# rgcgithub/regenie

Measured on AMD Instinct MI355X. Metric: Step-1 SNPs x samples x phenos / sec, higher is better.
Workload: dtype fp4 (exact integer Gram) + i8 (exact fixed-point digit planes of the fp64 operands: G~X / G~Y, many-row predictions) + f64 (solves, level 1); 1 GPU; BASELINE configs[1]: synthetic PLINK bed 50000 samples x 100000 SNPs (100000 per GPU), 1 QT pheno, bsize 1000, 22 chromosomes, 5-fold CV, 5x5 ridge grid; `value` is the HBM-resident figure (packed genotypes generated on the device, timed region = level 0 + level 1 + LOCO rows); the complete run from files on disk is `end_to_end_from_files`; samples=50000, snps=100000, phenos=1, bsize=1000, blocks=109, parallelism=blocks sharded x1, all-gather of W, level-1 Gram tiles / ridge systems shared x1

## Files before the change

### regenie_amd/csrc/l1.hip

```cpp
#include <algorithm>
#include <climits>
#include <cmath>
#include <cstdint>
#include <vector>
#include "rg_internal.h"

#define CT 64

struct L1Rows {
  const double* W; const double* y; const double* zero;
  int64_t Np; int L, P, p, n64;
};
__device__ __forceinline__ const double* l1_row(const L1Rows& R, int row) {
  if (row < R.L) return R.W + ((int64_t)row * R.P + R.p) * R.Np;
  if (row == R.n64) return R.y;
  return R.zero;
}

struct L1G64 {
  L1Rows R; int T, rtot, nslice, ntile, world, rank;
  double* out; int64_t slice_stride;
};
__global__ __launch_bounds__(256, 2) void k_l1_gram64(L1G64 g, SegLayout seg) {
  const int lane = threadIdx.x & 63, wave = threadIdx.x >> 6;
  const int f = blockIdx.y;
  const int item = blockIdx.x * 4 + wave;
  if (item >= g.ntile * g.nslice) return;
  const int sl = item / g.ntile, idx = item % g.ntile;
  if (idx % g.world != g.rank) return;
  int tc = 0, rem = idx;
  while (rem >= g.T + 1 - tc) { rem -= g.T + 1 - tc; ++tc; }
  const int tr = tc + rem;
  const int i = lane & 15, q = lane >> 4;
  const int64_t nch = seg.plen[f] / 64;
  const int64_t c0 = nch * sl / g.nslice, c1 = nch * (sl + 1) / g.nslice;
  const int64_t p0 = seg.pos_start[f] + 2 * q;
  const double* A[4];
  const double* B[4];
#pragma unroll
  for (int m = 0; m < 4; ++m) {
    A[m] = l1_row(g.R, tr * CT + m * 16 + i) + p0;
    B[m] = l1_row(g.R, tc * CT + m * 16 + i) + p0;
  }
  v4d acc[4][4];
// ... 93 lines not shown
    if (s + 1 < ns) issue((s + 1) & 1);
    if (live) {
      double2 a[4][2], b[4][2];
#pragma unroll
      for (int m = 0; m < 4; ++m) {
        a[m][0] = *reinterpret_cast<const double2*>(cur + oa + m * 2048);
        a[m][1] = *reinterpret_cast<const double2*>(cur + oa + m * 2048 + o4);
        b[m][0] = *reinterpret_cast<const double2*>(cur + ob + m * 2048);
        b[m][1] = *reinterpret_cast<const double2*>(cur + ob + m * 2048 + o4);
      }
#pragma unroll
      for (int kk = 0; kk < 4; ++kk)
#pragma unroll
        for (int m = 0; m < 4; ++m)
#pragma unroll
          for (int n = 0; n < 4; ++n) {
            const double av = kk == 0 ? a[m][0].x : (kk == 1 ? a[m][0].y : (kk == 2 ? a[m][1].x : a[m][1].y));
            const double bv = kk == 0 ? b[n][0].x : (kk == 1 ? b[n][0].y : (kk == 2 ? b[n][1].x : b[n][1].y));
            acc[m][n] = __builtin_amdgcn_mfma_f64_16x16x4f64(av, bv, acc[m][n], 0, 0, 0);
          }
    }
    asm volatile("s_waitcnt vmcnt(0) lgkmcnt(0)\n\ts_barrier" ::: "memory");
  }
  if (!live) return;
  double* O = g.out + (int64_t)it.slice * g.slice_stride + (int64_t)f * g.rtot * n64 + (int64_t)row0 * n64 + col0;
#pragma unroll
  for (int m = 0; m < 4; ++m)
#pragma unroll
    for (int n = 0; n < 4; ++n)
#pragma unroll
      for (int r = 0; r < 4; ++r) O[(int64_t)(m * 16 + q + 4 * r) * n64 + n * 16 + i] = acc[m][n][r];
}

__global__ __launch_bounds__(256) void k_l1_wty(L1Rows R, SegLayout seg, int rtot, int world, int rank, double* out) {
  __shared__ double red[4];
  const int l = blockIdx.x, f = blockIdx.y;
  if (l % world != rank) return;
  const double* w = R.W + ((int64_t)l * R.P + R.p) * R.Np + seg.pos_start[f];
  const double* y = R.y + seg.pos_start[f];
  const int64_t n = seg.plen[f];
  double t0 = 0.0, t1 = 0.0;
  for (int64_t e = 2 * (int64_t)threadIdx.x; e < n; e += 512) {
    const double2 wv = *reinterpret_cast<const double2*>(w + e), yv = *reinterpret_cast<const double2*>(y + e);
    t0 = fma(wv.x, yv.x, t0);
    t1 = fma(wv.y, yv.y, t1);
  }
  double t = t0 + t1;
  for (int o = 32; o > 0; o >>= 1) t += __shfl_down(t, o);
  if ((threadIdx.x & 63) == 0) red[threadIdx.x >> 6] = t;
  __syncthreads();
  if (threadIdx.x == 0) out[(int64_t)f * rtot * R.n64 + (int64_t)R.n64 * R.n64 + l] = (red[0] + red[1]) + (red[2] + red[3]);
}

static std::vector<L1Item> l1_build_items(int n64, int K, int nslice, int world, int rank) {
  const int T2 = (n64 + 127) / 128, S = 4, TS = (T2 + S - 1) / S;
  std::vector<std::vector<L1Item>> xl(8);
  int gi = 0;
  for (int f = 0; f < K; ++f)
    for (int sl = 0; sl < nslice; ++sl)
      for (int Mr = 0; Mr < TS; ++Mr)
        for (int Mc = 0; Mc <= Mr; ++Mc) {
          std::vector<L1Item>& dst = xl[gi % 8];
          bool any = false;
          for (int mr = Mr * S; mr < std::min(T2, (Mr + 1) * S); ++mr)
            for (int mc = Mc * S; mc < std::min(T2, (Mc + 1) * S); ++mc) {
              if (mc > mr) continue;
              if ((mr * (mr + 1) / 2 + mc) % world != rank) continue;
              dst.push_back(L1Item{(int16_t)mr, (int16_t)mc, (int16_t)f, (int16_t)sl});
              any = true;
            }
          if (any) ++gi;
        }
  size_t mx = 0;
  for (auto& v : xl) mx = std::max(mx, v.size());
  std::vector<L1Item> items(mx * 8, L1Item{0, 0, -1, 0});
  for (int x = 0; x < 8; ++x)
    for (size_t j = 0; j < xl[x].size(); ++j) items[8 * j + x] = xl[x][j];
  return items;
}

void rg_launch_fold_gram_rows(hipStream_t st, const double* G, int64_t ld, int L, int n64, int rtot, const double* zero,
                              const SegLayout& seg, double* out) {
  L1G64 g;
  g.R = L1Rows{G, zero, zero, ld, L, 1, 0, n64};
  g.T = n64 / CT; g.rtot = rtot; g.nslice = 1; g.ntile = g.T * (g.T + 1) / 2 + g.T; g.world = 1; g.rank = 0;
  g.out = out; g.slice_stride = 0;
  hipLaunchKernelGGL(k_l1_gram64, dim3((g.ntile + 3) / 4, seg.nseg), dim3(256), 0, st, g, seg);
}

__global__ void k_reduce_slices(const double* part, int64_t slice_stride, int nslice, int64_t n, double* out) {
  const int64_t e = (int64_t)blockIdx.x * blockDim.x + threadIdx.x;
  if (e >= n) return;
  double t = 0.0;
  for (int s = 0; s < nslice; ++s) t += part[(int64_t)s * slice_stride + e];
  out[e] = t;
}

__global__ void k_sum_folds(const double* fold, int64_t msz, int nfold, double* sum) {
  const int64_t e = (int64_t)blockIdx.x * blockDim.x + threadIdx.x;
  if (e >= msz) return;
  double t = 0.0;
  for (int f = 0; f < nfold; ++f) t += fold[(int64_t)f * msz + e];
  sum[e] = t;
}

__global__ __launch_bounds__(256) void k_loco(const double* pred, int nchr, int64_t N, const int32_t* chrom, int nchrom,
                                              double* out) {
  const int64_t n = (int64_t)blockIdx.x * 256 + threadIdx.x;
  if (n >= N) return;
  double tot = 0.0;
  for (int k = 0; k < nchr; ++k) tot += pred[(int64_t)k * N + n];
  for (int c = 0; c < nchrom; ++c) out[(int64_t)c * N + n] = tot;
  for (int k = 0; k < nchr; ++k) out[(int64_t)(chrom[k] - 1) * N + n] = tot - pred[(int64_t)k * N + n];
}

int rg_emit_pred(rg_ctx* ctx, hipStream_t st, const double* d_pred, int nchr, int p, double* pred_out) {
  const int64_t N = ctx->N;
  if (ctx->loco_nchrom <= 0) {
    RG_HIP(hipMemcpyAsync(pred_out + (int64_t)p * nchr * N, d_pred, sizeof(double) * (size_t)nchr * N, hipMemcpyDeviceToHost, st));
    return RG_OK;
  }
  if ((int)ctx->loco_chrom.size() != nchr) { ctx->err = "LOCO output: rg_set_loco_output was given a different number of chromosomes"; return RG_ERR_ARG; }
  const int nchrom = ctx->loco_nchrom;
  double* d_out = (double*)rg_ws(ctx, 11, sizeof(double) * (size_t)nchrom * N + sizeof(int32_t) * (size_t)nchr + 64);
  if (!d_out) { ctx->err = "LOCO output: out of device memory"; return RG_ERR_HIP; }
  int32_t* d_chr = reinterpret_cast<int32_t*>(d_out + (size_t)nchrom * N);
  RG_HIP(hipMemcpyAsync(d_chr, ctx->loco_chrom.data(), sizeof(int32_t) * nchr, hipMemcpyHostToDevice, st));
  hipLaunchKernelGGL(k_loco, dim3((unsigned)((N + 255) / 256)), dim3(256), 0, st, d_pred, nchr, N, d_chr, nchrom, d_out);
  RG_HIP(hipMemcpyAsync(pred_out + (int64_t)p * nchrom * N, d_out, sizeof(double) * (size_t)nchrom * N, hipMemcpyDeviceToHost, st));
  return RG_OK;
}

__global__ __launch_bounds__(256) void k_tiles_pack(double* fold, int64_t msz, int T, int n64, double* packed, int unpack) {
  const int t = blockIdx.x, f = blockIdx.y;
  int tr = (int)((sqrtf(8.0f * t + 1.0f) - 1.0f) * 0.5f);
  while ((tr + 1) * (tr + 2) / 2 <= t) ++tr;
  while (tr * (tr + 1) / 2 > t) --tr;
  int tc = t - tr * (tr + 1) / 2;
  if (tr >= T) { tc = t - T * (T + 1) / 2; tr = T; }
  double* src = fold + (int64_t)f * msz + (int64_t)tr * CT * n64 + tc * CT;
  double* pk = packed + ((int64_t)f * gridDim.x + t) * (CT * CT);
  for (int e = threadIdx.x; e < CT * CT; e += 256) {
    const int r = e >> 6, c = e & 63;
    if (unpack) src[(int64_t)r * n64 + c] = pk[e];
    else pk[e] = src[(int64_t)r * n64 + c];
  }
}

#define R1MAX 8
#define L1_CT 256
__global__ __launch_bounds__(256) void k_l1_cv(L1Rows R, const double* alpha , int R1,
                                               const int32_t* chunk_seg, const int64_t* chunk_pos,
                                               const int64_t* chunk_len, double* part) {
  __shared__ double sA[L1_CT][R1MAX];
  __shared__ double sred[4][R1MAX * 3 + 2];
  const int ch = blockIdx.x;
  const int f = chunk_seg[ch];
  const int64_t p0 = chunk_pos[ch], plen = chunk_len[ch];
  double tot[R1MAX * 3 + 2];
#pragma unroll
  for (int t = 0; t < R1MAX * 3 + 2; ++t) tot[t] = 0.0;
  for (int64_t sub = 0; sub < plen; sub += 256) {
// ... 14 lines not shown
        const int cn = min(L1_CT, R.L - c0);
        const double* w = R.W + ((int64_t)c0 * R.P + R.p) * R.Np + pos;
        for (int c = 0; c < cn; ++c) {
          const double x = w[(int64_t)c * R.P * R.Np];
#pragma unroll
          for (int j = 0; j < R1MAX; ++j) acc[j] = fma(x, sA[c][j], acc[j]);
        }
      }
    }
    if (live) {
      const double y = R.y[pos];
#pragma unroll
      for (int j = 0; j < R1MAX; ++j) {
        tot[3 * j] += acc[j];
        tot[3 * j + 1] = fma(acc[j], acc[j], tot[3 * j + 1]);
        tot[3 * j + 2] = fma(acc[j], y, tot[3 * j + 2]);
      }
      tot[R1MAX * 3] += y;
      tot[R1MAX * 3 + 1] = fma(y, y, tot[R1MAX * 3 + 1]);
    }
  }
#pragma unroll
  for (int t = 0; t < R1MAX * 3 + 2; ++t) {
    double x = tot[t];
    for (int o = 32; o > 0; o >>= 1) x += __shfl_down(x, o);
    if ((threadIdx.x & 63) == 0) sred[threadIdx.x >> 6][t] = x;
  }
  __syncthreads();
  if (threadIdx.x < R1MAX * 3 + 2)
    part[(int64_t)ch * (R1MAX * 3 + 2) + threadIdx.x] =
        (sred[0][threadIdx.x] + sred[1][threadIdx.x]) + (sred[2][threadIdx.x] + sred[3][threadIdx.x]);
}

__global__ __launch_bounds__(256) void k_l1_pred(L1Rows R, const double* alpha , int R1,
                                                 int best, const int32_t* chunk_seg,
                                                 const int64_t* chunk_pos, const int64_t* chunk_len,
                                                 const int32_t* chr_col0 , int nchr,
                                                 const int32_t* cidx, int64_t N, double* pred) {
  extern __shared__ double sAl[];
  const int ch = blockIdx.x;
  const int f = chunk_seg[ch];
  const int64_t p0 = chunk_pos[ch], plen = chunk_len[ch];
  const double* al = alpha + ((int64_t)f * R1 + best) * R.n64;
  for (int c = threadIdx.x; c < R.L; c += 256) sAl[c] = al[c];
  __syncthreads();
  for (int64_t sub = 0; sub < plen; sub += 256) {
    const int64_t pos = p0 + sub + threadIdx.x;
    if (sub + threadIdx.x >= plen) continue;
    const int32_t n = cidx[pos];
    if (n < 0) continue;
    for (int c = 0; c < nchr; ++c) {
      double acc = 0.0;
      const double* w = R.W + ((int64_t)chr_col0[c] * R.P + R.p) * R.Np + pos;
      const int nn = chr_col0[c + 1] - chr_col0[c];
      for (int t = 0; t < nn; ++t) acc = fma(w[(int64_t)t * R.P * R.Np], sAl[chr_col0[c] + t], acc);
      pred[(int64_t)c * N + n] = acc;
    }
  }
}

int rg_l1_qt_impl(rg_ctx* ctx, int R1, const double* tau, int nchr, const int32_t* cols_per_chr,
                  double* cumsum_out, int32_t* best_out, double* pred_out) {
  if (!ctx->have_problem || !(ctx->d_W || ctx->v_W)) { ctx->err = "rg_l1_qt: no level-0 predictors"; return RG_ERR_STATE; }
  if (R1 < 1 || R1 > R1MAX) { ctx->err = "rg_l1_qt: n_ridge_l1 must be in [1,8]"; return RG_ERR_ARG; }
  if (ctx->loocv) { ctx->err = "rg_l1_qt: the problem was set up for LOOCV (use rg_l1_qt_loocv)"; return RG_ERR_STATE; }
  hipStream_t st = ctx->stream;
  const int L = ctx->B_total * ctx->R0, K = ctx->K;
  if (!ctx->v_W && ctx->w_nb != ctx->B_total) { ctx->err = "rg_l1_qt: W holds a block range only (rg_set_block_range): level 1 needs the exchanged view"; return RG_ERR_STATE; }
  const double* Wv = ctx->v_W ? ctx->v_W : ctx->d_W;
  const int Pv = ctx->v_W ? ctx->v_np : ctx->P, P = ctx->v_np, p0v = ctx->v_p0;
  int ltot = 0;
  std::vector<int32_t> col0(nchr + 1, 0);
  for (int c = 0; c < nchr; ++c) { col0[c + 1] = col0[c] + cols_per_chr[c]; }
  ltot = col0[nchr];
  if (ltot != L) { ctx->err = "rg_l1_qt: cols_per_chr does not sum to n_blocks*R0"; return RG_ERR_ARG; }
  const int n64 = (int)rg_round_up(L, CT), rtot = n64 + CT, T = n64 / CT;
  const int64_t msz = (int64_t)rtot * n64;
  const int nsys = K * R1;
  const int nch = ctx->n_c256;
  const int NPART = R1MAX * 3 + 2;
  const int world = ctx->coll_world, rank = ctx->coll_rank;
  const bool multi = ctx->coll_allreduce != nullptr;
  const int b0 = multi ? (int)((int64_t)nsys * rank / world) : 0;
  const int b1 = multi ? (int)((int64_t)nsys * (rank + 1) / world) : nsys;
  const int nloc = b1 - b0;
  const int ntile = T * (T + 1) / 2 + T;
  int64_t min_nch = INT64_MAX;
  for (int f = 0; f < K; ++f) min_nch = std::min(min_nch, ctx->seg.plen[f] / 64);
  const int T2 = (n64 + 127) / 128, ntile2 = T2 * (T2 + 1) / 2;
  int nslice = (int)std::min<int64_t>(16, std::max<int64_t>(1, (3072 + (int64_t)ntile2 * K - 1) / ((int64_t)ntile2 * K)));
  nslice = (int)std::max<int64_t>(1, std::min<int64_t>(nslice, min_nch / 2));

  double *d_fold = nullptr, *d_part = nullptr, *d_sum = nullptr, *d_wk = nullptr, *d_dinv = nullptr, *d_tau = nullptr,
         *d_cvp = nullptr, *d_pred = nullptr, *d_alpha = nullptr, *d_pack = nullptr;
  int32_t* d_col0 = nullptr;
#define L1_WS(var, slot, type, count)                                                   \
  var = (type*)rg_ws(ctx, slot, sizeof(type) * (size_t)(count));                        \
  if (!var) { ctx->err = "rg_l1_qt: out of device memory"; return RG_ERR_HIP; }
  L1_WS(d_fold, 0, double, msz * K)
  if (nslice > 1) { L1_WS(d_part, 1, double, msz * K * nslice) }
  L1_WS(d_sum, 2, double, msz)
  L1_WS(d_wk, 3, double, msz * std::max(1, nloc))
  L1_WS(d_dinv, 4, double, rg_chol_ws_doubles((size_t)std::max(1, nloc), n64))
  L1_WS(d_tau, 5, double, R1)
  L1_WS(d_cvp, 6, double, (size_t)nch * NPART)
  L1_WS(d_pred, 7, double, (size_t)nchr * ctx->N)
  L1_WS(d_alpha, 8, double, (size_t)nsys * n64)
  L1_WS(d_col0, 9, int32_t, nchr + 1)
  if (multi) { L1_WS(d_pack, 10, double, (size_t)ntile * K * CT * CT) }
  L1Item* d_items = nullptr;
  const std::vector<L1Item> items = l1_build_items(n64, K, nslice, multi ? world : 1, multi ? rank : 0);
  L1_WS(d_items, 12, L1Item, items.size())
  RG_HIP(hipMemcpyAsync(d_items, items.data(), sizeof(L1Item) * items.size(), hipMemcpyHostToDevice, st));
  RG_HIP(hipStreamSynchronize(st));
#undef L1_WS
  RG_HIP(hipMemcpyAsync(d_col0, col0.data(), sizeof(int32_t) * (nchr + 1), hipMemcpyHostToDevice, st));
  std::vector<double> hpart((size_t)nch * NPART);
  int rc = RG_OK;
  auto lap = [&](double* slot, hipEvent_t e0, hipEvent_t e1) {
    if (!ctx->timing) return;
    hipEventRecord(e1, st); hipEventSynchronize(e1);
    float ms; hipEventElapsedTime(&ms, e0, e1); *slot += ms;
    hipEventRecord(e0, st);
  };

  for (int p = 0; p < P && rc == RG_OK; ++p) {
    const int pg = p0v + p, pw = ctx->v_W ? p : pg;
    L1Rows R{Wv, ctx->d_V + (int64_t)(ctx->C + pg) * ctx->Np, ctx->d_zero, ctx->Np, L, Pv, pw, n64};
    hipEvent_t e0 = ctx->ev0, e1 = ctx->ev1;
    if (ctx->timing) hipEventRecord(e0, st);
    double* gout = nslice > 1 ? d_part : d_fold;
    hipMemsetAsync(gout, 0, sizeof(double) * msz * K * nslice, st);
    L1G128 g{R, rtot, nslice, d_items, gout, msz * K};
    hipLaunchKernelGGL(k_l1_gram128, dim3((unsigned)items.size()), dim3(256), 0, st, g, ctx->seg);
    if (nslice > 1)
      hipLaunchKernelGGL(k_reduce_slices, dim3((unsigned)((msz * K + 255) / 256)), dim3(256), 0, st, d_part, msz * K,
                         nslice, msz * K, d_fold);
    hipLaunchKernelGGL(k_l1_wty, dim3(L, K), dim3(256), 0, st, R, ctx->seg, rtot, multi ? world : 1, multi ? rank : 0, d_fold);
    if (multi) {
      hipLaunchKernelGGL(k_tiles_pack, dim3(ntile, K), dim3(256), 0, st, d_fold, msz, T, n64, d_pack, 0);
      RG_HIP(hipStreamSynchronize(st));
      if (ctx->coll_allreduce(ctx->coll_user, d_pack, (int64_t)ntile * K * CT * CT) != 0) { ctx->err = "rg_l1_qt: all-reduce callback failed"; rc = RG_ERR_STATE; break; }
      hipLaunchKernelGGL(k_tiles_pack, dim3(ntile, K), dim3(256), 0, st, d_fold, msz, T, n64, d_pack, 1);
    }
    hipLaunchKernelGGL(k_sum_folds, dim3((unsigned)((msz + 255) / 256)), dim3(256), 0, st, d_fold, msz, K, d_sum);
    lap(&ctx->tm.ms_l1_gram, e0, e1);
    hipMemcpyAsync(d_tau, tau + (int64_t)p * R1, sizeof(double) * R1, hipMemcpyHostToDevice, st);
    hipMemsetAsync(d_alpha, 0, sizeof(double) * (size_t)nsys * n64, st);
    if (nloc > 0) {
      rg_launch_chol_solve_formed_x(st, d_sum, 0, d_fold, msz, K, d_tau, R1, nullptr, L, 1, d_wk, msz, n64, CT, 1,
                                    d_dinv, ctx->d_info + 1, &ctx->tm.n_chol_launches, 1, nullptr, 0, 0, 1, b0, nloc);
      RG_HIP(hipMemcpy2DAsync(d_alpha + (int64_t)b0 * n64, sizeof(double) * n64, d_wk + (int64_t)n64 * n64,
                              sizeof(double) * msz, sizeof(double) * n64, nloc, hipMemcpyDeviceToDevice, st));
    }
    if (multi) {
      RG_HIP(hipStreamSynchronize(st));
      if (ctx->coll_allreduce(ctx->coll_user, d_alpha, (int64_t)nsys * n64) != 0) { ctx->err = "rg_l1_qt: all-reduce callback failed"; rc = RG_ERR_STATE; break; }
    }
    lap(&ctx->tm.ms_l1_chol, e0, e1);
    hipLaunchKernelGGL(k_l1_cv, dim3(nch), dim3(256), 0, st, R, d_alpha, R1, ctx->d_c256_seg,
                       ctx->d_c256_pos, ctx->d_c256_len, d_cvp);
    RG_HIP(hipMemcpyAsync(hpart.data(), d_cvp, sizeof(double) * hpart.size(), hipMemcpyDeviceToHost, st));
    RG_HIP(hipStreamSynchronize(st));
    double* cs = cumsum_out + (int64_t)p * 5 * R1;
    for (int t = 0; t < 5 * R1; ++t) cs[t] = 0.0;
    double sy = 0.0, sy2 = 0.0;
    for (int ch = 0; ch < nch; ++ch) {
      const double* q = hpart.data() + (size_t)ch * NPART;
      for (int j = 0; j < R1; ++j) {
        cs[0 * R1 + j] += q[3 * j];
        cs[2 * R1 + j] += q[3 * j + 1];
        cs[4 * R1 + j] += q[3 * j + 2];
      }
      sy += q[R1MAX * 3];
      sy2 += q[R1MAX * 3 + 1];
    }
    for (int j = 0; j < R1; ++j) { cs[1 * R1 + j] = sy; cs[3 * R1 + j] = sy2; }
    int best = 0; double minv = 1e10;
    for (int j = 0; j < R1; ++j) {
      const double perf = (cs[2 * R1 + j] + cs[3 * R1 + j] - 2 * cs[4 * R1 + j]) / ctx->neff[pg];
      if (perf < minv) { best = j; minv = perf; }
    }
    best_out[p] = best;
    hipMemsetAsync(d_pred, 0, sizeof(double) * (size_t)nchr * ctx->N, st);
    hipLaunchKernelGGL(k_l1_pred, dim3(nch), dim3(256), sizeof(double) * L, st, R, d_alpha, R1, best,
                       ctx->d_c256_seg, ctx->d_c256_pos, ctx->d_c256_len, d_col0, nchr,
                       ctx->d_cidx, ctx->N, d_pred);
    if ((rc = rg_emit_pred(ctx, st, d_pred, nchr, p, pred_out))) break;
    RG_HIP(hipStreamSynchronize(st));
    if (ctx->timing) { hipEventRecord(e1, st); hipEventSynchronize(e1); float ms; hipEventElapsedTime(&ms, e0, e1); ctx->tm.ms_l1_pred += ms; }
    int32_t info[2] = {0, 0};
    RG_HIP(hipMemcpy(info, ctx->d_info, sizeof(info), hipMemcpyDeviceToHost));
    if (info[1]) { ctx->err = "level 1 ridge system is not positive definite"; rc = RG_ERR_NOT_SPD; }
  }
  return rc;
}
```

### regenie_amd/csrc/rg_api.hip

```cpp
#include <algorithm>
#include <cstdlib>
#include <cstring>
#include <chrono>
#include "rg_internal.h"

namespace {

template <class T>
int dev_alloc(rg_ctx* ctx, T** p, size_t n) {
  if (*p) { hipFree(*p); *p = nullptr; }
  if (n == 0) n = 1;
  RG_HIP(hipMalloc((void**)p, n * sizeof(T)));
  return RG_OK;
}
template <class T>
int dev_upload(rg_ctx* ctx, T** p, const std::vector<T>& v) {
  int rc = dev_alloc(ctx, p, v.size());
  if (rc) return rc;
  if (!v.empty()) RG_HIP(hipMemcpy(*p, v.data(), v.size() * sizeof(T), hipMemcpyHostToDevice));
  return RG_OK;
}

void free_all(rg_ctx* c) {
  void* ptrs[] = {c->d_cidx, c->d_act, c->d_V, c->d_maskp, c->d_Q, c->d_XtY, c->d_lambda, c->d_neff,
                  c->d_keptp, c->d_posc, c->d_zero, c->d_raw, c->d_pk, c->d_pk4, c->d_mu, c->d_nmiss,
                  c->d_xypart, c->d_chunk_seg, c->d_chunk_pos, c->d_chunk_len, c->d_S, c->d_F, c->d_Bm,
                  c->d_BQ, c->d_GYt, c->d_sc, c->d_fold, c->d_sum, c->d_wk, c->d_dinv, c->d_beta,
                  c->d_cb, c->d_psum, c->d_pstat, c->d_info, c->d_bs, c->d_blockid, (void*)c->d_rawptr, c->d_c1k_seg, c->d_c1k_pos,
                  c->d_c1k_len, c->d_c256_seg, c->d_c256_pos, c->d_c256_len, c->d_gt, c->d_zt, c->d_triws, c->d_lpart, c->d_bplanes, c->d_bsc, c->d_pkT, c->d_vd, c->d_vsc, c->d_xyS, c->d_segid};
  for (void* p : ptrs)
    if (p) hipFree(p);
  if (c->own_W && c->d_W) hipFree(c->d_W);
  for (int i = 0; i < 16; ++i)
    if (c->ws_ptr[i]) { hipFree(c->ws_ptr[i]); c->ws_ptr[i] = nullptr; c->ws_bytes[i] = 0; }
  for (int i = 0; i < 10; ++i)
    if (c->f64_ptr[i]) { hipFree(c->f64_ptr[i]); c->f64_ptr[i] = nullptr; c->f64_bytes[i] = 0; }
}

struct StageTimer {
  rg_ctx* c; double* slot;
  StageTimer(rg_ctx* ctx, double* s) : c(ctx), slot(s) { if (c->timing) hipEventRecord(c->ev0, c->stream); }
  ~StageTimer() {
    if (!c->timing) return;
    hipEventRecord(c->ev1, c->stream);
    hipEventSynchronize(c->ev1);
    float ms = 0;
    hipEventElapsedTime(&ms, c->ev0, c->ev1);
    *slot += ms;
  }
};

}

extern "C" {

int rg_create(rg_ctx** out, int device_id, void* hip_stream) {
  if (!out) return RG_ERR_ARG;
  *out = nullptr;
  int ndev = 0;
  if (hipGetDeviceCount(&ndev) != hipSuccess || ndev <= 0 || device_id >= ndev) return RG_ERR_HIP;
  if (hipSetDevice(device_id) != hipSuccess) return RG_ERR_HIP;
  rg_ctx* c = new rg_ctx();
  c->device = device_id;
  if (hip_stream) c->stream = (hipStream_t)hip_stream;
  else {
    if (hipStreamCreate(&c->stream) != hipSuccess) { delete c; return RG_ERR_HIP; }
    c->own_stream = true;
// ... 851 lines not shown
```

### regenie_amd/csrc/rg_internal.h

```cpp
#pragma once
#include <hip/hip_runtime.h>
#include <stdint.h>
#include <functional>
#include <string>
#include <vector>

#include "../../include/rg_step1.h"

#define RG_MAX_SEG 32
#define RG_TILE_G 128
#define RG_TILE_C 64

typedef int v4i __attribute__((ext_vector_type(4)));
typedef int v16i __attribute__((ext_vector_type(16)));
typedef double v4d __attribute__((ext_vector_type(4)));

static inline int64_t rg_round_up(int64_t x, int64_t m) { return (x + m - 1) / m * m; }
static inline size_t rg_chol_ws_doubles(size_t batch, int n64) {
  const size_t T = (size_t)n64 / 64;
  return batch * (T + (T + 3) / 4 * 10) * 4096;
}

struct SegLayout {
  int32_t nseg;
// ... 100 lines not shown
  uint8_t* d_pkT = nullptr;
  double* d_psum = nullptr;
  double* d_pstat = nullptr;
  int32_t* d_info = nullptr;
  int32_t* d_bs = nullptr;
  int32_t* d_blockid = nullptr;
  const uint8_t** d_rawptr = nullptr;
  std::vector<const uint8_t*> h_rawptr;
  std::vector<int> block_done;

  const double* v_W = nullptr;
  int v_p0 = 0, v_np = 0;

  int loco_nchrom = 0;
  std::vector<int32_t> loco_chrom;

  int coll_world = 1, coll_rank = 0;
  rg_allreduce_fn coll_allreduce = nullptr;
  void* coll_user = nullptr;

  rg_ctx* twin = nullptr;
  int n_pipe = 1;
  bool is_child = false;
  hipEvent_t ev_tw_fork = nullptr, ev_tw_join = nullptr;
  bool join_pending = false;
  int pipe_rr = 0;

  hipEvent_t ev_ingest = nullptr;
  bool ingest_pending = false;

  void* ws_ptr[16] = {};
  size_t ws_bytes[16] = {};

  void* f64_ptr[10] = {};
  size_t f64_bytes[10] = {};

  bool timing = false;
  rg_timing tm{};
  hipEvent_t ev0 = nullptr, ev1 = nullptr;
};

static inline double* rg_w_base(const rg_ctx* c) { return c->d_W ? c->d_W - (int64_t)c->w_b0 * c->R0 * c->P * c->Np : nullptr; }

static inline void* rg_ws(rg_ctx* ctx, int slot, size_t bytes) {
  if (bytes == 0) bytes = 8;
  if (ctx->ws_bytes[slot] < bytes) {
    if (ctx->ws_ptr[slot]) hipFree(ctx->ws_ptr[slot]);
    ctx->ws_ptr[slot] = nullptr; ctx->ws_bytes[slot] = 0;
    if (hipMalloc(&ctx->ws_ptr[slot], bytes) != hipSuccess) return nullptr;
    ctx->ws_bytes[slot] = bytes;
  }
  return ctx->ws_ptr[slot];
}

#if defined(__HIPCC__)
__device__ __forceinline__ void glds16(const void* sbase, uint32_t voff, uint32_t lds_addr) {
  const uint64_t a = reinterpret_cast<uint64_t>(sbase);
  const uint64_t sa = ((uint64_t)(uint32_t)__builtin_amdgcn_readfirstlane((int)(a >> 32)) << 32) |
                      (uint32_t)__builtin_amdgcn_readfirstlane((int)a);
  asm volatile("s_mov_b32 m0, %2\n\ts_nop 0\n\tglobal_load_lds_dwordx4 %0, %1" ::"v"(voff), "s"(sa),
               "s"(__builtin_amdgcn_readfirstlane((int)lds_addr))
               : "memory", "m0");
}

__device__ __forceinline__ void glds16p(const void* gptr, uint32_t lds_addr) {
  asm volatile("s_mov_b32 m0, %1\n\ts_nop 0\n\tglobal_load_lds_dwordx4 %0, off" ::"v"(gptr),
// ... 72 lines not shown
                     double* part);
#define RG_XY_LUT_DOSAGE 0x00010002u
#define RG_XY_LUT_SQUARE 0x00010004u
void rg_launch_xy_i8_sums(hipStream_t st, const uint8_t* pk, int64_t pk_ld, const int32_t* d_bs, const int32_t* nmiss, int ncols, int n128,
                          const SegLayout& seg, const int8_t* vd, int64_t Np, unsigned lut0, int32_t* S32);
void rg_launch_xy_i8_both(hipStream_t st, const uint8_t* pk, int64_t pk_ld, const int32_t* d_bs, int ncols, int n128, const SegLayout& seg,
                          const int8_t* vd, int64_t Np, unsigned lut0, int32_t* S32);
void rg_launch_xy_i8_planes(hipStream_t st, const int8_t* aplanes, int64_t a_set_stride, int nset, const int32_t* d_bs, int ncols, int n128,
                            const SegLayout& seg, const int8_t* vd, int64_t Np, int32_t* S32);
void rg_launch_l0_pred_i8(hipStream_t st, const PredArgs& a, const ChunkTab& c256, int pg, int ngrp, int8_t* planes, double* psc,
                          uint8_t* pkT);
void rg_launch_w_gather(hipStream_t st, const double* W, int64_t Np, int P, int p, int col0, int R0,
                        const int64_t* posc, int64_t N, double* out);
void rg_launch_w_scatter(hipStream_t st, double* W, int64_t Np, int P, int p, int col0, int R0,
                         const int64_t* posc, int64_t N, const double* in);
struct LoocvArgs {
  int nblk, R0, P, C, n128, n64, rtot, row_g0;
  int64_t Np, pk_ld, pk_blk_stride;
  const uint8_t* pk; const double* mu; const double* sc; const double* Bm; const double* V;
  const double* maskp; const double* neff; const int32_t* bs; const int32_t* blockid;
  const double* wk; double* gt; double* W;
  int64_t gt_pos0 = 0, gt_len = 0;
};
size_t rg_loocv_tri_ws_doubles(int nblk, int n64, int P, int R0);
int rg_l0_loocv_tri(rg_ctx* ctx, hipStream_t st, const LoocvArgs& la, int max_bs, const double* d_sum, int rtot, double* ws, double* zt,
                    int64_t chunk, const std::function<void(int64_t, int64_t)>& gt_chunk);
void rg_launch_decode_gt(hipStream_t st, const LoocvArgs& a);
void rg_launch_l0_loocv(hipStream_t st, const LoocvArgs& a, double* part0, double* part1, int nchunk);
void rg_launch_fold_gram_rows(hipStream_t st, const double* G, int64_t ld, int L, int n64, int rtot, const double* zero,
                              const SegLayout& seg, double* out);
int rg_l0_blocks_f64_impl(rg_ctx* ctx, int nblk, const int32_t* block_ids, const int32_t* bs, const double* const* rows,
                          int64_t row_stride, int mem_kind);
int rg_emit_pred(rg_ctx* ctx, hipStream_t st, const double* d_pred, int nchr, int p, double* pred_out);
struct L1Args;
int rg_l1_qt_impl(rg_ctx* ctx, int R1, const double* tau, int nchr, const int32_t* cols_per_chr,
                  double* cumsum_out, int32_t* best_out, double* pred_out);
#define RG_WGRAM_FP16 1
#define RG_WGRAM_BF16X3 2
int rg_launch_wgram_bf16(rg_ctx* ctx, hipStream_t st, const double* W, int64_t Np, int L, int P, int p, int n64, const double* wv, double* sw, int nchain,
                         const int32_t* d_chainmap, const int32_t* h_chainmap, int nslot, int excl_own, double* part, int64_t out_stride,
                         int max_slices, int fmt);
int rg_l1_qt_loocv_impl(rg_ctx* ctx, int R1, const double* tau, int nchr, const int32_t* cols_per_chr,
                        double* cumsum_out, int32_t* best_out, double* pred_out);
int rg_l1_cox_impl(rg_ctx* ctx, int pheno, int R1, const double* time, const double* event, const double* offset, const rg_cox_options* opt,
                   int nchr, const int32_t* cols_per_chr, double* tau_out, double* deviance_out, int32_t* converged_out, int32_t* best_out,
                   double* pred_out);
int rg_l1_bt_impl(rg_ctx* ctx, int R1, const double* tau, const double* yraw, const double* offset,
                  const rg_bt_options* opt, int nchr, const int32_t* cols_per_chr, double* cumsum_out,
                  int32_t* converged_out, int32_t* best_out, double* pred_out);
```

Baseline: 168.0 billion SNP*sample*pheno/s.

## Move level-1 CV selection on device, fuse reductions, cache items, pin host buffers

Level-1 QT now does the per-chunk CV sum and best-lambda choice in a new device kernel instead of copying partials to the host. It folds slice reduction, W'y, and fold sums into one k_l1_reduce launch with no pre-memset. When L is small it pads n64 to 128 and puts y in the padding row, dropping the extra 64-row block. It also caches the work-item list across calls and stages uploads and downloads through pinned host buffers, which removes several blocking syncs. The cost is more complex code paths, and the gram kernel must still fully overwrite the output it no longer zeroes.

```diff
diff --git a/regenie_amd/csrc/l1.hip b/regenie_amd/csrc/l1.hip
--- a/regenie_amd/csrc/l1.hip
+++ b/regenie_amd/csrc/l1.hip
@@ -7,9 +7,20 @@
 
 #define CT 64
 
+static void* rg_hpin(rg_ctx* ctx, int slot, size_t bytes) {
+  if (bytes == 0) bytes = 8;
+  if (ctx->hpin_bytes[slot] < bytes) {
+    if (ctx->hpin_ptr[slot]) hipHostFree(ctx->hpin_ptr[slot]);
+    ctx->hpin_ptr[slot] = nullptr; ctx->hpin_bytes[slot] = 0;
+    if (hipHostMalloc(&ctx->hpin_ptr[slot], bytes, hipHostMallocDefault) != hipSuccess) return nullptr;
+    ctx->hpin_bytes[slot] = bytes;
+  }
+  return ctx->hpin_ptr[slot];
+}
+
 struct L1Rows {
   const double* W; const double* y; const double* zero;
-  int64_t Np; int L, P, p, n64;
+  int64_t Np; int L, P, p, n64, yrow;
 };
 __device__ __forceinline__ const double* l1_row(const L1Rows& R, int row) {
   if (row < R.L) return R.W + ((int64_t)row * R.P + R.p) * R.Np;
@@ -169,24 +180,52 @@
       for (int r = 0; r < 4; ++r) O[(int64_t)(m * 16 + q + 4 * r) * n64 + n * 16 + i] = acc[m][n][r];
 }
 
-__global__ __launch_bounds__(256) void k_l1_wty(L1Rows R, SegLayout seg, int rtot, int world, int rank, double* out) {
+__global__ __launch_bounds__(256) void k_l1_reduce(L1Rows R, SegLayout seg, int rtot, int K, int nslice, const double* part,
+                                                   int64_t slice_stride, int world, int rank, double* fold, double* sum) {
+  const int n64 = R.n64;
+  const int64_t msz = (int64_t)rtot * n64;
+  if ((int)blockIdx.x < rtot) {
+    const int i = blockIdx.x;
+    const int mr = i >> 7;
+    for (int c = threadIdx.x; c < n64; c += 256) {
+      if (i == R.yrow && c < R.L) continue;
+      const int64_t e = (int64_t)i * n64 + c;
+      const int mc = c >> 7;
+      const bool have = i < n64 && (c >> 6) <= (i >> 6) && (mr * (mr + 1) / 2 + mc) % world == rank;
+      double tot = 0.0;
+      for (int f = 0; f < K; ++f) {
+        double t = 0.0;
+        if (have) {
+          const double* q = part + (int64_t)f * msz + e;
+          for (int s = 0; s < nslice; ++s) t += q[(int64_t)s * slice_stride];
+        }
+        if (!have || part != fold) fold[(int64_t)f * msz + e] = t;
+        tot += t;
+      }
+      if (sum) sum[e] = tot;
+    }
+    return;
+  }
   __shared__ double red[4];
-  const int l = blockIdx.x, f = blockIdx.y;
-  if (l % world != rank) return;
-  const double* w = R.W + ((int64_t)l * R.P + R.p) * R.Np + seg.pos_start[f];
-  const double* y = R.y + seg.pos_start[f];
-  const int64_t n = seg.plen[f];
-  double t0 = 0.0, t1 = 0.0;
-  for (int64_t e = 2 * (int64_t)threadIdx.x; e < n; e += 512) {
-    const double2 wv = *reinterpret_cast<const double2*>(w + e), yv = *reinterpret_cast<const double2*>(y + e);
-    t0 = fma(wv.x, yv.x, t0);
-    t1 = fma(wv.y, yv.y, t1);
-  }
-  double t = t0 + t1;
-  for (int o = 32; o > 0; o >>= 1) t += __shfl_down(t, o);
-  if ((threadIdx.x & 63) == 0) red[threadIdx.x >> 6] = t;
-  __syncthreads();
-  if (threadIdx.x == 0) out[(int64_t)f * rtot * R.n64 + (int64_t)R.n64 * R.n64 + l] = (red[0] + red[1]) + (red[2] + red[3]);
+  const int l = (blockIdx.x - rtot) / K, f = (blockIdx.x - rtot) % K;
+  double v = 0.0;
+  if (l % world == rank) {
+    const double* w = R.W + ((int64_t)l * R.P + R.p) * R.Np + seg.pos_start[f];
+    const double* y = R.y + seg.pos_start[f];
+    const int64_t n = seg.plen[f];
+    double t0 = 0.0, t1 = 0.0;
+    for (int64_t e = 2 * (int64_t)threadIdx.x; e < n; e += 512) {
+      const double2 wv = *reinterpret_cast<const double2*>(w + e), yv = *reinterpret_cast<const double2*>(y + e);
+      t0 = fma(wv.x, yv.x, t0);
+      t1 = fma(wv.y, yv.y, t1);
+    }
+    double t = t0 + t1;
+    for (int o = 32; o > 0; o >>= 1) t += __shfl_down(t, o);
+    if ((threadIdx.x & 63) == 0) red[threadIdx.x >> 6] = t;
+    __syncthreads();
+    v = (red[0] + red[1]) + (red[2] + red[3]);
+  }
+  if (threadIdx.x == 0) fold[(int64_t)f * msz + (int64_t)R.yrow * n64 + l] = v;
 }
 
 static std::vector<L1Item> l1_build_items(int n64, int K, int nslice, int world, int rank) {
@@ -219,23 +258,15 @@
 void rg_launch_fold_gram_rows(hipStream_t st, const double* G, int64_t ld, int L, int n64, int rtot, const double* zero,
                               const SegLayout& seg, double* out) {
   L1G64 g;
-  g.R = L1Rows{G, zero, zero, ld, L, 1, 0, n64};
+  g.R = L1Rows{G, zero, zero, ld, L, 1, 0, n64, n64};
   g.T = n64 / CT; g.rtot = rtot; g.nslice = 1; g.ntile = g.T * (g.T + 1) / 2 + g.T; g.world = 1; g.rank = 0;
   g.out = out; g.slice_stride = 0;
   hipLaunchKernelGGL(k_l1_gram64, dim3((g.ntile + 3) / 4, seg.nseg), dim3(256), 0, st, g, seg);
 }
 
-__global__ void k_reduce_slices(const double* part, int64_t slice_stride, int nslice, int64_t n, double* out) {
+__global__ void k_sum_folds(const double* fold, int64_t msz, int64_t n, int nfold, double* sum) {
   const int64_t e = (int64_t)blockIdx.x * blockDim.x + threadIdx.x;
   if (e >= n) return;
-  double t = 0.0;
-  for (int s = 0; s < nslice; ++s) t += part[(int64_t)s * slice_stride + e];
-  out[e] = t;
-}
-
-__global__ void k_sum_folds(const double* fold, int64_t msz, int nfold, double* sum) {
-  const int64_t e = (int64_t)blockIdx.x * blockDim.x + threadIdx.x;
-  if (e >= msz) return;
   double t = 0.0;
   for (int f = 0; f < nfold; ++f) t += fold[(int64_t)f * msz + e];
   sum[e] = t;
@@ -252,9 +283,13 @@
 }
 
 int rg_emit_pred(rg_ctx* ctx, hipStream_t st, const double* d_pred, int nchr, int p, double* pred_out) {
+  return rg_emit_pred_rows(ctx, st, d_pred, nchr, pred_out + (int64_t)p * rg_pred_rows(ctx, nchr) * ctx->N);
+}
+
+int rg_emit_pred_rows(rg_ctx* ctx, hipStream_t st, const double* d_pred, int nchr, double* rows_out) {
   const int64_t N = ctx->N;
   if (ctx->loco_nchrom <= 0) {
-    RG_HIP(hipMemcpyAsync(pred_out + (int64_t)p * nchr * N, d_pred, sizeof(double) * (size_t)nchr * N, hipMemcpyDeviceToHost, st));
+    RG_HIP(hipMemcpyAsync(rows_out, d_pred, sizeof(double) * (size_t)nchr * N, hipMemcpyDeviceToHost, st));
     return RG_OK;
   }
   if ((int)ctx->loco_chrom.size() != nchr) { ctx->err = "LOCO output: rg_set_loco_output was given a different number of chromosomes"; return RG_ERR_ARG; }
@@ -264,7 +299,7 @@
   int32_t* d_chr = reinterpret_cast<int32_t*>(d_out + (size_t)nchrom * N);
   RG_HIP(hipMemcpyAsync(d_chr, ctx->loco_chrom.data(), sizeof(int32_t) * nchr, hipMemcpyHostToDevice, st));
   hipLaunchKernelGGL(k_loco, dim3((unsigned)((N + 255) / 256)), dim3(256), 0, st, d_pred, nchr, N, d_chr, nchrom, d_out);
-  RG_HIP(hipMemcpyAsync(pred_out + (int64_t)p * nchrom * N, d_out, sizeof(double) * (size_t)nchrom * N, hipMemcpyDeviceToHost, st));
+  RG_HIP(hipMemcpyAsync(rows_out, d_out, sizeof(double) * (size_t)nchrom * N, hipMemcpyDeviceToHost, st));
   return RG_OK;
 }
 
@@ -345,8 +380,37 @@
         (sred[0][threadIdx.x] + sred[1][threadIdx.x]) + (sred[2][threadIdx.x] + sred[3][threadIdx.x]);
 }
 
+#define L1_NPART (R1MAX * 3 + 2)
+__global__ __launch_bounds__(256) void k_l1_select(const double* part, int nch, int R1, const double* neff, double* cs,
+                                                   int32_t* best, const int32_t* info, int32_t* flags) {
+  __shared__ double buf[64 * L1_NPART];
+  __shared__ double tot[L1_NPART];
+  double t = 0.0;
+  for (int c0 = 0; c0 < nch; c0 += 64) {
+    const int n = min(64, nch - c0) * L1_NPART;
+    __syncthreads();
+    for (int e = threadIdx.x; e < n; e += 256) buf[e] = part[(int64_t)c0 * L1_NPART + e];
+    __syncthreads();
+    if (threadIdx.x < L1_NPART)
+      for (int e = threadIdx.x; e < n; e += L1_NPART) t += buf[e];
+  }
+  if (threadIdx.x < L1_NPART) tot[threadIdx.x] = t;
+  __syncthreads();
+  if (threadIdx.x != 0) return;
+  int b = 0;
+  double minv = 1e10;
+  for (int j = 0; j < R1; ++j) {
+    const double sx = tot[3 * j], sx2 = tot[3 * j + 1], sxy = tot[3 * j + 2], sy = tot[R1MAX * 3], sy2 = tot[R1MAX * 3 + 1];
+    cs[0 * R1 + j] = sx; cs[1 * R1 + j] = sy; cs[2 * R1 + j] = sx2; cs[3 * R1 + j] = sy2; cs[4 * R1 + j] = sxy;
+    const double perf = (sx2 + sy2 - 2 * sxy) / neff[0];
+    if (perf < minv) { b = j; minv = perf; }
+  }
+  best[0] = b;
+  flags[0] = info[0]; flags[1] = info[1];
+}
+
 __global__ __launch_bounds__(256) void k_l1_pred(L1Rows R, const double* alpha , int R1,
-                                                 int best, const int32_t* chunk_seg,
+                                                 const int32_t* best_sel, const int32_t* chunk_seg,
                                                  const int64_t* chunk_pos, const int64_t* chunk_len,
                                                  const int32_t* chr_col0 , int nchr,
                                                  const int32_t* cidx, int64_t N, double* pred) {
@@ -354,7 +418,7 @@
   const int ch = blockIdx.x;
   const int f = chunk_seg[ch];
   const int64_t p0 = chunk_pos[ch], plen = chunk_len[ch];
-  const double* al = alpha + ((int64_t)f * R1 + best) * R.n64;
+  const double* al = alpha + ((int64_t)f * R1 + best_sel[0]) * R.n64;
   for (int c = threadIdx.x; c < R.L; c += 256) sAl[c] = al[c];
   __syncthreads();
   for (int64_t sub = 0; sub < plen; sub += 256) {
@@ -371,6 +435,9 @@
     }
   }
 }
+
+#define L1_P128_MAX_L 640
+static inline bool l1_use_p128(int L) { return L <= L1_P128_MAX_L; }
 
 int rg_l1_qt_impl(rg_ctx* ctx, int R1, const double* tau, int nchr, const int32_t* cols_per_chr,
                   double* cumsum_out, int32_t* best_out, double* pred_out) {
@@ -387,26 +454,31 @@
   for (int c = 0; c < nchr; ++c) { col0[c + 1] = col0[c] + cols_per_chr[c]; }
   ltot = col0[nchr];
   if (ltot != L) { ctx->err = "rg_l1_qt: cols_per_chr does not sum to n_blocks*R0"; return RG_ERR_ARG; }
-  const int n64 = (int)rg_round_up(L, CT), rtot = n64 + CT, T = n64 / CT;
+  const bool p128 = l1_use_p128(L);
+  const int n64 = p128 ? (int)rg_round_up(L + 1, 128) : (int)rg_round_up(L, CT);
+  const int rtot = p128 ? n64 : n64 + CT, yrow = p128 ? L : n64, T = n64 / CT;
   const int64_t msz = (int64_t)rtot * n64;
   const int nsys = K * R1;
   const int nch = ctx->n_c256;
-  const int NPART = R1MAX * 3 + 2;
+  const int NPART = L1_NPART;
   const int world = ctx->coll_world, rank = ctx->coll_rank;
   const bool multi = ctx->coll_allreduce != nullptr;
   const int b0 = multi ? (int)((int64_t)nsys * rank / world) : 0;
   const int b1 = multi ? (int)((int64_t)nsys * (rank + 1) / world) : nsys;
   const int nloc = b1 - b0;
-  const int ntile = T * (T + 1) / 2 + T;
+  const int ntile = T * (T + 1) / 2 + (p128 ? 0 : T);
   int64_t min_nch = INT64_MAX;
   for (int f = 0; f < K; ++f) min_nch = std::min(min_nch, ctx->seg.plen[f] / 64);
   const int T2 = (n64 + 127) / 128, ntile2 = T2 * (T2 + 1) / 2;
   int nslice = (int)std::min<int64_t>(16, std::max<int64_t>(1, (3072 + (int64_t)ntile2 * K - 1) / ((int64_t)ntile2 * K)));
   nslice = (int)std::max<int64_t>(1, std::min<int64_t>(nslice, min_nch / 2));
 
-  double *d_fold = nullptr, *d_part = nullptr, *d_sum = nullptr, *d_wk = nullptr, *d_dinv = nullptr, *d_tau = nullptr,
+  double *d_fold = nullptr, *d_part = nullptr, *d_sum = nullptr, *d_wk = nullptr, *d_dinv = nullptr, *d_par = nullptr,
          *d_cvp = nullptr, *d_pred = nullptr, *d_alpha = nullptr, *d_pack = nullptr;
   int32_t* d_col0 = nullptr;
+  const size_t up_d = (size_t)P * R1, up_i = (size_t)nchr + 2, dn_d = (size_t)P * 5 * R1, dn_i = (size_t)P + 2;
+  const size_t up_bytes = sizeof(double) * up_d + sizeof(int32_t) * up_i, dn_bytes = sizeof(double) * dn_d + sizeof(int32_t) * dn_i;
+  const size_t dn_off = rg_round_up((int64_t)up_bytes, 64);
 #define L1_WS(var, slot, type, count)                                                   \
   var = (type*)rg_ws(ctx, slot, sizeof(type) * (size_t)(count));                        \
   if (!var) { ctx->err = "rg_l1_qt: out of device memory"; return RG_ERR_HIP; }
@@ -415,20 +487,57 @@
   L1_WS(d_sum, 2, double, msz)
   L1_WS(d_wk, 3, double, msz * std::max(1, nloc))
   L1_WS(d_dinv, 4, double, rg_chol_ws_doubles((size_t)std::max(1, nloc), n64))
-  L1_WS(d_tau, 5, double, R1)
+  L1_WS(d_par, 5, double, (dn_off + dn_bytes + 7) / 8)
   L1_WS(d_cvp, 6, double, (size_t)nch * NPART)
   L1_WS(d_pred, 7, double, (size_t)nchr * ctx->N)
   L1_WS(d_alpha, 8, double, (size_t)nsys * n64)
-  L1_WS(d_col0, 9, int32_t, nchr + 1)
   if (multi) { L1_WS(d_pack, 10, double, (size_t)ntile * K * CT * CT) }
+  uint8_t* h_par = (uint8_t*)rg_hpin(ctx, 1, dn_off + dn_bytes);
+  if (!h_par) { ctx->err = "rg_l1_qt: out of page-locked host memory"; return RG_ERR_HIP; }
+  double* d_tau = d_par;
+  d_col0 = reinterpret_cast<int32_t*>(d_par + up_d);
+  const int32_t* d_L = d_col0 + nchr + 1;
+  double* d_cs = reinterpret_cast<double*>(reinterpret_cast<uint8_t*>(d_par) + dn_off);
+  int32_t* d_best = reinterpret_cast<int32_t*>(d_cs + dn_d);
+  int32_t* d_flags = d_best + P;
+  {
+    double* h_tau = reinterpret_cast<double*>(h_par);
+    int32_t* h_col0 = reinterpret_cast<int32_t*>(h_tau + up_d);
+    std::copy(tau, tau + up_d, h_tau);
+    std::copy(col0.begin(), col0.end(), h_col0);
+    h_col0[nchr + 1] = L;
+    RG_HIP(hipMemcpyAsync(d_par, h_par, up_bytes, hipMemcpyHostToDevice, st));
+  }
   L1Item* d_items = nullptr;
-  const std::vector<L1Item> items = l1_build_items(n64, K, nslice, multi ? world : 1, multi ? rank : 0);
-  L1_WS(d_items, 12, L1Item, items.size())
-  RG_HIP(hipMemcpyAsync(d_items, items.data(), sizeof(L1Item) * items.size(), hipMemcpyHostToDevice, st));
-  RG_HIP(hipStreamSynchronize(st));
+  {
+    const int key[5] = {n64, K, nslice, multi ? world : 1, multi ? rank : 0};
+    if (!std::equal(key, key + 5, ctx->l1_item_key) || !ctx->ws_ptr[12]) {
+      const std::vector<L1Item> items = l1_build_items(n64, K, nslice, key[3], key[4]);
+      L1Item* h_items = (L1Item*)rg_hpin(ctx, 0, sizeof(L1Item) * items.size());
+      if (!h_items) { ctx->err = "rg_l1_qt: out of page-locked host memory"; return RG_ERR_HIP; }
+      std::copy(items.begin(), items.end(), h_items);
+      ctx->l1_item_key[0] = -1;
+      L1_WS(d_items, 12, L1Item, items.size())
+      RG_HIP(hipMemcpyAsync(d_items, h_items, sizeof(L1Item) * items.size(), hipMemcpyHostToDevice, st));
+      std::copy(key, key + 5, ctx->l1_item_key);
+      ctx->l1_item_count = (int)items.size();
+    }
+    d_items = (L1Item*)ctx->ws_ptr[12];
+  }
+  const unsigned nitems = (unsigned)ctx->l1_item_count;
 #undef L1_WS
-  RG_HIP(hipMemcpyAsync(d_col0, col0.data(), sizeof(int32_t) * (nchr + 1), hipMemcpyHostToDevice, st));
-  std::vector<double> hpart((size_t)nch * NPART);
+  const int64_t prow = (int64_t)rg_pred_rows(ctx, nchr) * ctx->N;
+  bool out_pinned = false;
+  {
+    hipPointerAttribute_t at{};
+    if (hipPointerGetAttributes(&at, pred_out) == hipSuccess) out_pinned = at.type == hipMemoryTypeHost;
+    else (void)hipGetLastError();
+  }
+  double* h_stage = nullptr;
+  if (!out_pinned) {
+    h_stage = (double*)rg_hpin(ctx, 2, sizeof(double) * (size_t)prow);
+    if (!h_stage) { ctx->err = "rg_l1_qt: out of page-locked host memory"; return RG_ERR_HIP; }
+  }
   int rc = RG_OK;
   auto lap = [&](double* slot, hipEvent_t e0, hipEvent_t e1) {
     if (!ctx->timing) return;
@@ -439,32 +548,35 @@
 
   for (int p = 0; p < P && rc == RG_OK; ++p) {
     const int pg = p0v + p, pw = ctx->v_W ? p : pg;
-    L1Rows R{Wv, ctx->d_V + (int64_t)(ctx->C + pg) * ctx->Np, ctx->d_zero, ctx->Np, L, Pv, pw, n64};
+    L1Rows R{Wv, ctx->d_V + (int64_t)(ctx->C + pg) * ctx->Np, ctx->d_zero, ctx->Np, L, Pv, pw, n64, yrow};
     hipEvent_t e0 = ctx->ev0, e1 = ctx->ev1;
     if (ctx->timing) hipEventRecord(e0, st);
     double* gout = nslice > 1 ? d_part : d_fold;
-    hipMemsetAsync(gout, 0, sizeof(double) * msz * K * nslice, st);
     L1G128 g{R, rtot, nslice, d_items, gout, msz * K};
-    hipLaunchKernelGGL(k_l1_gram128, dim3((unsigned)items.size()), dim3(256), 0, st, g, ctx->seg);
-    if (nslice > 1)
-      hipLaunchKernelGGL(k_reduce_slices, dim3((unsigned)((msz * K + 255) / 256)), dim3(256), 0, st, d_part, msz * K,
-                         nslice, msz * K, d_fold);
-    hipLaunchKernelGGL(k_l1_wty, dim3(L, K), dim3(256), 0, st, R, ctx->seg, rtot, multi ? world : 1, multi ? rank : 0, d_fold);
+    hipLaunchKernelGGL(k_l1_gram128, dim3(nitems), dim3(256), 0, st, g, ctx->seg);
+    hipLaunchKernelGGL(k_l1_reduce, dim3(rtot + L * K), dim3(256), 0, st, R, ctx->seg, rtot, K, nslice, gout, msz * K,
+                       multi ? world : 1, multi ? rank : 0, d_fold, multi ? nullptr : d_sum);
+    if (!multi)
+      hipLaunchKernelGGL(k_sum_folds, dim3((unsigned)((L + 255) / 256)), dim3(256), 0, st, d_fold + (int64_t)yrow * n64, msz, (int64_t)L, K,
+                         d_sum + (int64_t)yrow * n64);
     if (multi) {
       hipLaunchKernelGGL(k_tiles_pack, dim3(ntile, K), dim3(256), 0, st, d_fold, msz, T, n64, d_pack, 0);
       RG_HIP(hipStreamSynchronize(st));
       if (ctx->coll_allreduce(ctx->coll_user, d_pack, (int64_t)ntile * K * CT * CT) != 0) { ctx->err = "rg_l1_qt: all-reduce callback failed"; rc = RG_ERR_STATE; break; }
       hipLaunchKernelGGL(k_tiles_pack, dim3(ntile, K), dim3(256), 0, st, d_fold, msz, T, n64, d_pack, 1);
-    }
-    hipLaunchKernelGGL(k_sum_folds, dim3((unsigned)((msz + 255) / 256)), dim3(256), 0, st, d_fold, msz, K, d_sum);
+      hipLaunchKernelGGL(k_sum_folds, dim3((unsigned)((msz + 255) / 256)), dim3(256), 0, st, d_fold, msz, msz, K, d_sum);
+    }
     lap(&ctx->tm.ms_l1_gram, e0, e1);
-    hipMemcpyAsync(d_tau, tau + (int64_t)p * R1, sizeof(double) * R1, hipMemcpyHostToDevice, st);
     hipMemsetAsync(d_alpha, 0, sizeof(double) * (size_t)nsys * n64, st);
     if (nloc > 0) {
-      rg_launch_chol_solve_formed_x(st, d_sum, 0, d_fold, msz, K, d_tau, R1, nullptr, L, 1, d_wk, msz, n64, CT, 1,
-                                    d_dinv, ctx->d_info + 1, &ctx->tm.n_chol_launches, 1, nullptr, 0, 0, 1, b0, nloc);
-      RG_HIP(hipMemcpy2DAsync(d_alpha + (int64_t)b0 * n64, sizeof(double) * n64, d_wk + (int64_t)n64 * n64,
-                              sizeof(double) * msz, sizeof(double) * n64, nloc, hipMemcpyDeviceToDevice, st));
+      if (p128)
+        rg_launch_chol_solve_formed_x(st, d_sum, 0, d_fold, msz, K, d_tau + (int64_t)p * R1, R1, d_L, L, 1, d_wk, msz, n64, 0, 1,
+                                      d_dinv, ctx->d_info + 1, &ctx->tm.n_chol_launches, 1, nullptr, 0, 0, 1, b0, nloc, 0, 1);
+      else
+        rg_launch_chol_solve_formed_x(st, d_sum, 0, d_fold, msz, K, d_tau + (int64_t)p * R1, R1, nullptr, L, 1, d_wk, msz, n64, CT, 1,
+                                      d_dinv, ctx->d_info + 1, &ctx->tm.n_chol_launches, 1, nullptr, 0, 0, 1, b0, nloc);
+      RG_HIP(hipMemcpy2DAsync(d_alpha + (int64_t)b0 * n64, sizeof(double) * n64, d_wk + (int64_t)yrow * n64,
+                              sizeof(double) * msz, sizeof(double) * L, nloc, hipMemcpyDeviceToDevice, st));
     }
     if (multi) {
       RG_HIP(hipStreamSynchronize(st));
@@ -473,38 +585,32 @@
     lap(&ctx->tm.ms_l1_chol, e0, e1);
     hipLaunchKernelGGL(k_l1_cv, dim3(nch), dim3(256), 0, st, R, d_alpha, R1, ctx->d_c256_seg,
                        ctx->d_c256_pos, ctx->d_c256_len, d_cvp);
-    RG_HIP(hipMemcpyAsync(hpart.data(), d_cvp, sizeof(double) * hpart.size(), hipMemcpyDeviceToHost, st));
-    RG_HIP(hipStreamSynchronize(st));
-    double* cs = cumsum_out + (int64_t)p * 5 * R1;
-    for (int t = 0; t < 5 * R1; ++t) cs[t] = 0.0;
-    double sy = 0.0, sy2 = 0.0;
-    for (int ch = 0; ch < nch; ++ch) {
-      const double* q = hpart.data() + (size_t)ch * NPART;
-      for (int j = 0; j < R1; ++j) {
-        cs[0 * R1 + j] += q[3 * j];
-        cs[2 * R1 + j] += q[3 * j + 1];
-        cs[4 * R1 + j] += q[3 * j + 2];
-      }
-      sy += q[R1MAX * 3];
-      sy2 += q[R1MAX * 3 + 1];
-    }
-    for (int j = 0; j < R1; ++j) { cs[1 * R1 + j] = sy; cs[3 * R1 + j] = sy2; }
-    int best = 0; double minv = 1e10;
-    for (int j = 0; j < R1; ++j) {
-      const double perf = (cs[2 * R1 + j] + cs[3 * R1 + j] - 2 * cs[4 * R1 + j]) / ctx->neff[pg];
-      if (perf < minv) { best = j; minv = perf; }
-    }
-    best_out[p] = best;
+    hipLaunchKernelGGL(k_l1_select, dim3(1), dim3(256), 0, st, d_cvp, nch, R1, ctx->d_neff + pg, d_cs + (int64_t)p * 5 * R1,
+                       d_best + p, ctx->d_info, d_flags);
     hipMemsetAsync(d_pred, 0, sizeof(double) * (size_t)nchr * ctx->N, st);
-    hipLaunchKernelGGL(k_l1_pred, dim3(nch), dim3(256), sizeof(double) * L, st, R, d_alpha, R1, best,
+    hipLaunchKernelGGL(k_l1_pred, dim3(nch), dim3(256), sizeof(double) * L, st, R, d_alpha, R1, d_best + p,
                        ctx->d_c256_seg, ctx->d_c256_pos, ctx->d_c256_len, d_col0, nchr,
                        ctx->d_cidx, ctx->N, d_pred);
-    if ((rc = rg_emit_pred(ctx, st, d_pred, nchr, p, pred_out))) break;
+    if ((rc = rg_emit_pred_rows(ctx, st, d_pred, nchr, out_pinned ? pred_out + p * prow : h_stage))) break;
+    if (!out_pinned) {
+      RG_HIP(hipStreamSynchronize(st));
+      std::copy(h_stage, h_stage + prow, pred_out + p * prow);
+    }
+    if (ctx->timing) { hipEventRecord(e1, st); hipEventSynchronize(e1); float ms; hipEventElapsedTime(&ms, e0, e1); ctx->tm.ms_l1_pred += ms; }
+  }
+  if (rc == RG_OK) {
+    RG_HIP(hipMemcpyAsync(h_par + dn_off, d_cs, dn_bytes, hipMemcpyDeviceToHost, st));
     RG_HIP(hipStreamSynchronize(st));
-    if (ctx->timing) { hipEventRecord(e1, st); hipEventSynchronize(e1); float ms; hipEventElapsedTime(&ms, e0, e1); ctx->tm.ms_l1_pred += ms; }
-    int32_t info[2] = {0, 0};
-    RG_HIP(hipMemcpy(info, ctx->d_info, sizeof(info), hipMemcpyDeviceToHost));
-    if (info[1]) { ctx->err = "level 1 ridge system is not positive definite"; rc = RG_ERR_NOT_SPD; }
+    const double* h_cs = reinterpret_cast<const double*>(h_par + dn_off);
+    const int32_t* h_best = reinterpret_cast<const int32_t*>(h_cs + dn_d);
+    std::copy(h_cs, h_cs + dn_d, cumsum_out);
+    std::copy(h_best, h_best + P, best_out);
+    if (h_best[P + 1]) {
+      ctx->err = "level 1 ridge system is not positive definite";
+      rc = RG_ERR_NOT_SPD;
+    }
+  } else {
+    (void)hipStreamSynchronize(st);
   }
   return rc;
 }
diff --git a/regenie_amd/csrc/rg_api.hip b/regenie_amd/csrc/rg_api.hip
--- a/regenie_amd/csrc/rg_api.hip
+++ b/regenie_amd/csrc/rg_api.hip
@@ -33,6 +33,9 @@
   if (c->own_W && c->d_W) hipFree(c->d_W);
   for (int i = 0; i < 16; ++i)
     if (c->ws_ptr[i]) { hipFree(c->ws_ptr[i]); c->ws_ptr[i] = nullptr; c->ws_bytes[i] = 0; }
+  for (int i = 0; i < 3; ++i)
+    if (c->hpin_ptr[i]) { hipHostFree(c->hpin_ptr[i]); c->hpin_ptr[i] = nullptr; c->hpin_bytes[i] = 0; }
+  c->l1_item_key[0] = -1; c->l1_item_count = 0;
   for (int i = 0; i < 10; ++i)
     if (c->f64_ptr[i]) { hipFree(c->f64_ptr[i]); c->f64_ptr[i] = nullptr; c->f64_bytes[i] = 0; }
 }
diff --git a/regenie_amd/csrc/rg_internal.h b/regenie_amd/csrc/rg_internal.h
--- a/regenie_amd/csrc/rg_internal.h
+++ b/regenie_amd/csrc/rg_internal.h
@@ -156,6 +156,11 @@
   void* ws_ptr[16] = {};
   size_t ws_bytes[16] = {};
 
+  int l1_item_key[5] = {-1, -1, -1, -1, -1};
+  int l1_item_count = 0;
+  void* hpin_ptr[3] = {};
+  size_t hpin_bytes[3] = {};
+
   void* f64_ptr[10] = {};
   size_t f64_bytes[10] = {};
 
@@ -294,6 +299,8 @@
 int rg_l0_blocks_f64_impl(rg_ctx* ctx, int nblk, const int32_t* block_ids, const int32_t* bs, const double* const* rows,
                           int64_t row_stride, int mem_kind);
 int rg_emit_pred(rg_ctx* ctx, hipStream_t st, const double* d_pred, int nchr, int p, double* pred_out);
+int rg_emit_pred_rows(rg_ctx* ctx, hipStream_t st, const double* d_pred, int nchr, double* rows_out);
+static inline int rg_pred_rows(const rg_ctx* ctx, int nchr) { return ctx->loco_nchrom > 0 ? ctx->loco_nchrom : nchr; }
 struct L1Args;
 int rg_l1_qt_impl(rg_ctx* ctx, int R1, const double* tau, int nchr, const int32_t* cols_per_chr,
                   double* cumsum_out, int32_t* best_out, double* pred_out);
```

New measurement: 169.2 billion SNP*sample*pheno/s (median of 5 runs). Within noise of the previous version (+0.7%).
